# funcwj/setk

Measured on AMD Instinct MI355X. Metric: real-time-factor (audio-sec/wall-sec), 8-ch 16 kHz MVDR, higher is better.
Workload: dtype f32; 1 GPU; 8-ch 16 kHz oracle-mask MVDR, 30 s utterances, 125 per GPU (BASELINE configs[2] shard: 1000 at 8 GPUs), STFT 512/256/hann/center, inputs resident in HBM; utts_per_gpu=125, channels=8, frames=1876, beamformer=mvdr, parallelism=utterance-sharded x1

## Files before the change

setk_amd/csrc/capi_fused.hip:

```cpp
#include "capi.h"

using namespace setk;

extern "C" {

int setk_apply_weights_batch(setk_handle_t h, int n_utts, int num_channels,
                             const float* const* audio, const int* num_samples,
                             const float* weights, int n_sets, const int* weight_index,
                             void* const* wave, int flags, void* stream) {
    if (!h || n_utts <= 0 || !audio || !num_samples || !weights || n_sets <= 0 || !wave)
        return fail(h, SETK_ERR_INVALID, "bad args");
    SETK_TRY(require_plan512(h));
    const int C = num_channels;
    if (C < 1 || C > kMaxChannels) return fail(h, SETK_ERR_UNSUPPORTED, "1 <= num_channels <= 8");
    if (weight_index)
        for (int u = 0; u < n_utts; ++u)
            if (weight_index[u] < 0 || weight_index[u] >= n_sets)
                return fail(h, SETK_ERR_INVALID, "weight index out of range");
    hipStream_t s;
    SETK_TRY(begin_call(h, stream, &s));
    const bool pcm16 = (flags & SETK_FLAG_OUT_PCM16) != 0;

    std::vector<UttDesc> uds = zeroed_utts(n_utts);
    std::vector<WorkItem> items;
// ... 122 lines not shown
    memcpy(blob.data() + b_ud + b_i1, items2.data(), b_i2);
    if (blob != h->desc_cache) {
        if (blob.size() > h->d_desc_cap) {
            HIP_TRY(h, hipStreamSynchronize(s));
            if (h->d_desc) (void)hipFree(h->d_desc);
            h->d_desc = nullptr;
            h->d_desc_cap = 0;
            HIP_TRY(h, hipMalloc(reinterpret_cast<void**>(&h->d_desc), blob.size() * 2));
            h->d_desc_cap = blob.size() * 2;
        }
        HIP_TRY(h, h2d_small(h, h->d_desc, blob.data(), blob.size(), s));
        h->desc_cache.swap(blob);
    }
    const UttDesc* d_uds = reinterpret_cast<const UttDesc*>(h->d_desc);
    const WorkItem* d_items1 = reinterpret_cast<const WorkItem*>(h->d_desc + b_ud);
    const WorkItem* d_items2 = reinterpret_cast<const WorkItem*>(h->d_desc + b_ud + b_i1);

    const int planes_out = mpdr ? 6 * NP : 4 * NP;
    float *d_part, *d_covar, *d_w;
    unsigned* d_small;
    SETK_TRY(arena_get(h, (size_t)nparts_total * nplanes_partial(C) * kBinsPad * 4, &d_part));
    SETK_TRY(arena_get(h, (size_t)n_utts * planes_out * kBinsPad * 4, &d_covar));
    SETK_TRY(arena_get(h, (size_t)n_utts * C * kBinsPad * 8, &d_w));
    SETK_TRY(arena_get(h, (size_t)n_utts * 3 * 4, &d_small));
    unsigned* d_norm = d_small;
    unsigned* d_omax = d_small + n_utts;
    int* d_status = reinterpret_cast<int*>(d_small + 2 * n_utts);
    HIP_TRY(h, hipMemsetAsync(d_small, 0, (size_t)n_utts * 3 * 4, s));

    SETK_TRY(profile_begin(h, s));

    Pass1Args p1 = pass1_args(h, d_uds, d_items1);
    p1.partials = d_part;
    p1.norm_bits = d_norm;
    p1.flags = opts->flags;
    p1.mc_tab = h->d_mc_tab;
    p1.mc_win = h->d_mc_win;
    const bool mc1 = !in_pcm && h->mc_enabled && pass1_mc_supported(C, g.hop) && getenv("SETK_MC_PASS1") &&
                     atoi(getenv("SETK_MC_PASS1")) != 0;
    if (in_pcm) p1.window = h->d_window_pcm;
    if (mc1)
        HIP_TRY(h, launch_pass1_mc(C, p1, (int)items1.size(), s));
    else
        HIP_TRY(h, launch_pass1(C, false, p1, (int)items1.size(), s, in_pcm));
    SETK_TRY(profile_mark(h, 1, s));
    FinalizeArgs fa;
    memset(&fa, 0, sizeof(fa));
    fa.utts = d_uds;
    fa.partials = d_part;
    fa.covar = d_covar;
    fa.num_channels = C;
    fa.with_ry = mpdr ? 1 : 0;
    fa.num_scale = mc1 ? (float)((h->mc_peak / 1024.0) * (h->mc_peak / 1024.0)) : 1.f;
    const bool fuse_reduce = !(taps && (taps->Rs || taps->Rn)) && max_parts <= 4 &&
                             !(kind == SETK_BF_PMWF && opts->pmwf_ref < 0) &&
                             !(getenv("SETK_FUSED_REDUCE") && atoi(getenv("SETK_FUSED_REDUCE")) == 0);
    if (!fuse_reduce) HIP_TRY(h, launch_finalize(fa, n_utts, s));
    OutBuf tap_rs, tap_rn, tap_w;
    if (taps && taps->Rs) {
        SETK_TRY(stage_out(h, taps->Rs, (size_t)n_utts * kBins * C * C * sizeof(float2), &tap_rs));
        HIP_TRY(h, launch_unpack_covar(d_covar, n_utts, planes_out, 0, kBins, C,
                                       static_cast<float*>(tap_rs.dev), s));
        SETK_TRY(copy_back(h, tap_rs, s));
    }
    if (taps && taps->Rn) {
        SETK_TRY(stage_out(h, taps->Rn, (size_t)n_utts * kBins * C * C * sizeof(float2), &tap_rn));
        HIP_TRY(h, launch_unpack_covar(d_covar, n_utts, planes_out, 2 * NP, kBins, C,
                                       static_cast<float*>(tap_rn.dev), s));
        SETK_TRY(copy_back(h, tap_rn, s));
    }

    SolveArgs sa;
    memset(&sa, 0, sizeof(sa));
    sa.covar = d_covar;
    sa.weight = d_w;
    sa.status = d_status;
    sa.n_utts = n_utts;
    sa.num_bins = kBins;
    sa.num_channels = C;
    sa.planes = planes_out;
    sa.kind = kind;
    sa.flags = opts->flags;
    sa.rank1 = opts->rank1;
    sa.pmwf_ref = opts->pmwf_ref;
    sa.pmwf_beta = opts->pmwf_beta;
    sa.partials = fuse_reduce ? d_part : nullptr;
    sa.utts = d_uds;
    sa.num_scale = fa.num_scale;
    if (kind == SETK_BF_PMWF && opts->pmwf_ref < 0) {
        SETK_TRY(arena_get(h, (size_t)n_utts * kBins * C * 2 * sizeof(double), &sa.snr_acc));
        SETK_TRY(arena_get(h, (size_t)n_utts * kBins * C * C * 8, &sa.wmat));
    }
    HIP_TRY(h, launch_solve(sa, s));
    if (kind == SETK_BF_PMWF && opts->pmwf_ref < 0) HIP_TRY(h, launch_pmwf_select(sa, nullptr, s));
    SETK_TRY(profile_mark(h, 2, s));
    if (taps && taps->weight) {
        SETK_TRY(stage_out(h, taps->weight, (size_t)n_utts * kBins * C * sizeof(float2), &tap_w));
        HIP_TRY(h, launch_unpack_weight_batch(d_w, n_utts, kBins, C,
                                              static_cast<float*>(tap_w.dev), s));
        SETK_TRY(copy_back(h, tap_w, s));
    }

    Pass2Args p2 = pass2_args(h, d_uds, d_items2, d_omax);
    p2.weight = d_w;
    p2.norm_bits = d_norm;
    p2.flags = opts->flags;
    p2.mc_tab = h->d_mc_tab;
// ... 20 lines not shown
```

setk_amd/csrc/common.h:

```cpp
#pragma once
#include <hip/hip_runtime.h>
#include <stdint.h>

namespace setk {

constexpr int kNfft = 512;
constexpr int kBins = 257;
constexpr int kBinsPad = 264;
constexpr int kMaxChannels = 8;
constexpr int kMaxChannels16 = 16;
constexpr int kSuperTile = 16;
constexpr int kPass2Threads = 16 * kSuperTile;
constexpr int kPass2WavesPerSimd = 2;
constexpr int kMaxKeep = 7;

__host__ __device__ constexpr int npairs(int c) { return c * (c + 1) / 2; }
__host__ __device__ constexpr int pass1_tile_frames(int c) { return (32 / c) < 8 ? (32 / c) : 8; }
__host__ __device__ constexpr int nplanes_partial(int c) { return 4 * npairs(c) + 2; }
__host__ __device__ constexpr int pair_index(int i, int j, int c) {
    return i * c - i * (i - 1) / 2 + (j - i);
}

constexpr int kAudioF32 = 0;
constexpr int kAudioPcm16 = 1;

struct UttDesc {
    const float* audio;
    const float* mask_s;
    const float* mask_n;
    float* wave_f32;
    void* wave_out;
    int num_samples;
    int num_frames;
    int out_len;
    int part0;
    int nparts;
    int audio_fmt;
    int ch_stride;
    int pad_;
};

struct WorkItem {
    int utt;
    int t0, t1;
    int part;
    int last;
};

struct StftGeom {
    int hop;
    int pad;
    int center;
    int keep;
};

struct Pass1Args {
    const UttDesc* utts;
    const WorkItem* items;
    float* partials;
    const float* window;
    const float2* tw256;
    const float2* tw512;
    unsigned* norm_bits;
    float* spec_dump;
    int dump_pitch;
    StftGeom g;
    int flags;
    const unsigned* mc_tab;
    const float* mc_win;
};

struct FinalizeArgs {
    const UttDesc* utts;
    const float* partials;
    float* covar;
    int num_channels;
    int with_ry;
    float num_scale;
};

struct SolveArgs {
    const float* covar;
    float* weight;
    int* status;
    int* bin_status;
    double* snr_acc;
    float* wmat;
    int n_utts;
    int num_bins;
    int num_channels;
    int planes;
    int kind, flags, rank1, pmwf_ref;
    float pmwf_beta;
// ... 184 lines not shown
```

setk_amd/csrc/dpp.h:

```cpp
#pragma once
#include <hip/hip_runtime.h>

namespace setk {

#ifndef SD
#define SD __device__ __forceinline__
#endif

template <int M>
SD int dpp_xor(int v) {
    constexpr int qp[4] = {0, 0xB1, 0x4E, 0x1B};
    if constexpr (M < 4) {
        return __builtin_amdgcn_update_dpp(0, v, qp[M], 0xf, 0xf, true);
    } else if constexpr (M == 7) {
        return __builtin_amdgcn_update_dpp(0, v, 0x141, 0xf, 0xf, true);
    } else if constexpr (M < 8) {
        const int h = __builtin_amdgcn_update_dpp(0, v, 0x141, 0xf, 0xf, true);
        return __builtin_amdgcn_update_dpp(0, h, qp[M ^ 7], 0xf, 0xf, true);
    } else if constexpr (M == 8) {
        return __builtin_amdgcn_update_dpp(0, v, 0x128, 0xf, 0xf, true);
    } else if constexpr (M < 12) {
        const int h = __builtin_amdgcn_update_dpp(0, v, 0x128, 0xf, 0xf, true);
        return __builtin_amdgcn_update_dpp(0, h, qp[M ^ 8], 0xf, 0xf, true);
    } else if constexpr (M == 15) {
        return __builtin_amdgcn_update_dpp(0, v, 0x140, 0xf, 0xf, true);
    } else {
        const int h = __builtin_amdgcn_update_dpp(0, v, 0x140, 0xf, 0xf, true);
        return __builtin_amdgcn_update_dpp(0, h, qp[M ^ 15], 0xf, 0xf, true);
    }
}
template <int M>
SD double dshfl_xor(double x) {
    const long long b = __builtin_bit_cast(long long, x);
    const int lo = dpp_xor<M>((int)(b & 0xffffffffll));
    const int hi = dpp_xor<M>((int)(b >> 32));
    return __builtin_bit_cast(double, ((long long)hi << 32) | (unsigned int)lo);
}

}
```

setk_amd/csrc/solve.hip:

```cpp
#include "common.h"
#include "dpp.h"
#include <hip/hip_runtime.h>
#include "../../include/setk_hip.h"

namespace setk {

typedef double2 cd;

#define SD __device__ __forceinline__

SD cd zadd(cd a, cd b) { return make_double2(a.x + b.x, a.y + b.y); }
SD cd zsub(cd a, cd b) { return make_double2(a.x - b.x, a.y - b.y); }
SD cd zmul(cd a, cd b) { return make_double2(a.x * b.x - a.y * b.y, a.x * b.y + a.y * b.x); }
SD cd zmulc(cd a, cd b) { return make_double2(a.x * b.x + a.y * b.y, a.y * b.x - a.x * b.y); }
SD cd zcmul(cd a, cd b) { return make_double2(a.x * b.x + a.y * b.y, a.x * b.y - a.y * b.x); }
SD cd zscale(cd a, double s) { return make_double2(a.x * s, a.y * s); }
SD cd zdiv(cd a, cd b) {
    const double d = b.x * b.x + b.y * b.y;
    return make_double2((a.x * b.x + a.y * b.y) / d, (a.y * b.x - a.x * b.y) / d);
}
SD double zabs2(cd a) { return a.x * a.x + a.y * a.y; }
template <int C> struct Grp { static constexpr int W = (C > 8) ? 16 : (C > 4) ? 8 : 4; };
template <int W>
SD cd zshfl(cd v, int src) { return make_double2(__shfl(v.x, src, W), __shfl(v.y, src, W)); }

constexpr int kKindPevd = 100;
constexpr double kEpsF32 = 1.1920928955078125e-07;

template <int C, int M>
SD bool jacobi_round(cd (&g)[C], int j, double floor2) {
    const double tol2 = 1e-16;
    const int p = j ^ M;
    cd gp[C];
    double m = 0.0, o = 0.0, dyb = 0.0;
    cd d = make_double2(0.0, 0.0);
#pragma unroll
    for (int i = 0; i < C; ++i) {
        gp[i] = make_double2(dshfl_xor<M>(g[i].x), dshfl_xor<M>(g[i].y));
        m = fma(g[i].x, g[i].x, fma(g[i].y, g[i].y, m));
        o = fma(gp[i].x, gp[i].x, fma(gp[i].y, gp[i].y, o));
        d.x = fma(g[i].x, gp[i].x, fma(g[i].y, gp[i].y, d.x));
        d.y = fma(g[i].x, gp[i].y, d.y);
        dyb = fma(g[i].y, gp[i].x, dyb);
    }
    d.y -= dyb;
    const double dd = fma(d.x, d.x, d.y * d.y);
    if (dd > tol2 * (m * o) && dd > floor2) {
        const double absd = sqrt(dd);
        const double sigma = (j < p) ? 1.0 : -1.0;
        const double zeta = sigma * (o - m) / (2.0 * absd);
        const double t = copysign(1.0, zeta) / (fabs(zeta) + sqrt(1.0 + zeta * zeta));
        const double cs = 1.0 / sqrt(1.0 + t * t);
        const double sn = cs * t;
        const double f = sigma * sn / absd;
        const cd ph = make_double2(d.x * f, -d.y * f);
#pragma unroll
        for (int i = 0; i < C; ++i) g[i] = zsub(zscale(g[i], cs), zmul(ph, gp[i]));
        return true;
    }
    return false;
}

template <int C>
SD void jacobi_pevd(cd (&g)[C], int j, cd (&out)[C], double& lam, int& noconv) {
    constexpr int W = Grp<C>::W;
    bool done = false;
    for (int sweep = 0; sweep < 40 && !done; ++sweep) {
        double mm = 0.0;
#pragma unroll
        for (int i = 0; i < C; ++i) mm += zabs2(g[i]);
#pragma unroll
        for (int sft = 1; sft < W; sft <<= 1) mm = fmax(mm, __shfl_xor(mm, sft, W));
        const double floor2 = 1e-28 * mm * mm;
        bool rot = false;
        rot |= jacobi_round<C, 1>(g, j, floor2);
        rot |= jacobi_round<C, 2>(g, j, floor2);
        rot |= jacobi_round<C, 3>(g, j, floor2);
        if constexpr (W >= 8) {
            rot |= jacobi_round<C, 4>(g, j, floor2);
            rot |= jacobi_round<C, 5>(g, j, floor2);
            rot |= jacobi_round<C, 6>(g, j, floor2);
            rot |= jacobi_round<C, 7>(g, j, floor2);
        }
        if constexpr (W == 16) {
            rot |= jacobi_round<C, 8>(g, j, floor2);
            rot |= jacobi_round<C, 9>(g, j, floor2);
            rot |= jacobi_round<C, 10>(g, j, floor2);
            rot |= jacobi_round<C, 11>(g, j, floor2);
            rot |= jacobi_round<C, 12>(g, j, floor2);
            rot |= jacobi_round<C, 13>(g, j, floor2);
            rot |= jacobi_round<C, 14>(g, j, floor2);
            rot |= jacobi_round<C, 15>(g, j, floor2);
        }
        done = !__any(rot);
    }
    if (!done) noconv = 1;
    double m = 0.0;
#pragma unroll
    for (int i = 0; i < C; ++i) m += zabs2(g[i]);
    double best = m;
    int bj = j;
#pragma unroll
    for (int s = 1; s < W; s <<= 1) {
        const double ob = __shfl_xor(best, s, W);
        const int oj = __shfl_xor(bj, s, W);
        if (ob > best || (ob == best && oj < bj)) {
            best = ob;
            bj = oj;
        }
    }
    lam = sqrt(best);
    const double inv = (lam > 0.0) ? 1.0 / lam : 0.0;
#pragma unroll
    for (int i = 0; i < C; ++i) {
        out[i] = zscale(zshfl<W>(g[i], bj), inv);
        if (!(lam > 0.0)) out[i] = make_double2((i == 0) ? 1.0 : 0.0, 0.0);
    }
}

template <int C>
SD void herm_matvec(const cd (&col)[C], const cd (&x)[C], cd (&y)[C]) {
    cd mine = make_double2(0.0, 0.0);
#pragma unroll
    for (int m = 0; m < C; ++m) mine = zadd(mine, zcmul(col[m], x[m]));
#pragma unroll
    for (int i = 0; i < C; ++i) y[i] = zshfl<Grp<C>::W>(mine, i);
}

template <int M>
SD float fxor(float x) {
    return __builtin_bit_cast(float, dpp_xor<M>(__builtin_bit_cast(int, x)));
}
template <int C, int M>
SD bool jacobi_round_f32(float2 (&g)[C], int j, float floor2) {
    const float tol2 = 1e-11f;
    const int p = j ^ M;
    float2 gp[C];
    float m = 0.f;
    float2 d = make_float2(0.f, 0.f);
    float dyb = 0.f;
#pragma unroll
    for (int i = 0; i < C; ++i) {
        gp[i] = make_float2(fxor<M>(g[i].x), fxor<M>(g[i].y));
        m = fmaf(g[i].x, g[i].x, fmaf(g[i].y, g[i].y, m));
        d.x = fmaf(g[i].x, gp[i].x, fmaf(g[i].y, gp[i].y, d.x));
        d.y = fmaf(g[i].x, gp[i].y, d.y);
        dyb = fmaf(g[i].y, gp[i].x, dyb);
    }
    d.y -= dyb;
    const float o = fxor<M>(m);
    const float dd = fmaf(d.x, d.x, d.y * d.y);
    if (dd > tol2 * (m * o) && dd > floor2) {
        const float rabs = __builtin_amdgcn_rsqf(dd);
        const float sigma = (j < p) ? 1.f : -1.f;
        const float zeta = sigma * (o - m) * 0.5f * rabs;
        const float t = copysignf(1.f, zeta) / (fabsf(zeta) + sqrtf(fmaf(zeta, zeta, 1.f)));
        const float cs = __builtin_amdgcn_rsqf(fmaf(t, t, 1.f));
        const float f = sigma * cs * t * rabs;
        const float2 ph = make_float2(d.x * f, -d.y * f);
#pragma unroll
        for (int i = 0; i < C; ++i) {
            const float2 t0 = g[i];
            g[i].x = fmaf(t0.x, cs, fmaf(-ph.x, gp[i].x, ph.y * gp[i].y));
            g[i].y = fmaf(t0.y, cs, fmaf(-ph.x, gp[i].y, -ph.y * gp[i].x));
        }
        return true;
    }
    return false;
}

template <int C>
SD void pevd_mixed(const cd (&a)[C], int j, cd (&out)[C], double& lam, int& noconv) {
    constexpr int W = Grp<C>::W;
    if constexpr (W > 8) {
        cd g[C];
#pragma unroll
        for (int i = 0; i < C; ++i) g[i] = a[i];
        jacobi_pevd<C>(g, j, out, lam, noconv);
        return;
    } else {
        double dg = 0.0;
#pragma unroll
        for (int i = 0; i < C; ++i)
            if (i == j) dg = a[i].x;
#pragma unroll
        for (int s = 1; s < W; s <<= 1) dg = fmax(dg, __shfl_xor(dg, s, W));
        const double rs = (dg > 0.0) ? 1.0 / dg : 0.0;
        float2 g[C];
#pragma unroll
        for (int i = 0; i < C; ++i) g[i] = make_float2((float)(a[i].x * rs), (float)(a[i].y * rs));
        bool done = false;
        for (int sweep = 0; sweep < 40 && !done; ++sweep) {
            float mm = 0.f;
#pragma unroll
            for (int i = 0; i < C; ++i) mm = fmaf(g[i].x, g[i].x, fmaf(g[i].y, g[i].y, mm));
            mm = fmaxf(mm, fxor<1>(mm));
            mm = fmaxf(mm, fxor<2>(mm));
            if constexpr (W == 8) mm = fmaxf(mm, fxor<4>(mm));
            const float floor2 = 1e-12f * mm * mm;
            bool rot = false;
            rot |= jacobi_round_f32<C, 1>(g, j, floor2);
            rot |= jacobi_round_f32<C, 2>(g, j, floor2);
            rot |= jacobi_round_f32<C, 3>(g, j, floor2);
            if constexpr (W == 8) {
                rot |= jacobi_round_f32<C, 4>(g, j, floor2);
                rot |= jacobi_round_f32<C, 5>(g, j, floor2);
                rot |= jacobi_round_f32<C, 6>(g, j, floor2);
                rot |= jacobi_round_f32<C, 7>(g, j, floor2);
            }
            done = !__any(rot);
        }
        if (!done) noconv = 1;
        float m = 0.f;
#pragma unroll
        for (int i = 0; i < C; ++i) m = fmaf(g[i].x, g[i].x, fmaf(g[i].y, g[i].y, m));
        float best = m;
        int bj = j;
#pragma unroll
        for (int s = 1; s < W; s <<= 1) {
            const float ob = __shfl_xor(best, s, W);
            const int oj = __shfl_xor(bj, s, W);
            if (ob > best || (ob == best && oj < bj)) {
                best = ob;
                bj = oj;
            }
        }
        cd v[C];
        double nn = 0.0;
#pragma unroll
        for (int i = 0; i < C; ++i) {
            v[i] = make_double2((double)__shfl(g[i].x, bj, W), (double)__shfl(g[i].y, bj, W));
            nn += zabs2(v[i]);
        }
        double inv = (nn > 0.0) ? 1.0 / sqrt(nn) : 0.0;
#pragma unroll
        for (int i = 0; i < C; ++i) v[i] = zscale(v[i], inv);
        const double nj = sqrt((double)m);
        const double ij = (nj > 0.0) ? 1.0 / nj : 0.0;
        const double theta_j = nj * dg;
        cd y[C];
#pragma unroll 1
        for (int it = 0; it < 2; ++it) {
            herm_matvec<C>(a, v, y);
            double theta = 0.0;
#pragma unroll
            for (int i = 0; i < C; ++i) theta += zcmul(v[i], y[i]).x;
            cd c = make_double2(0.0, 0.0);
#pragma unroll
            for (int i = 0; i < C; ++i) {
                const cd u = make_double2((double)g[i].x * ij, (double)g[i].y * ij);
                c = zadd(c, zcmul(u, zsub(y[i], zscale(v[i], theta))));
            }
            const double den = theta - theta_j;
            const bool use = j != bj && nj > 0.0 && fabs(den) > 16.0 * kEpsF32 * fabs(theta);
            const cd coef = use ? zscale(c, 1.0 / den) : make_double2(0.0, 0.0);
            nn = 0.0;
#pragma unroll
            for (int i = 0; i < C; ++i) {
                cd t = zmul(make_double2((double)g[i].x * ij, (double)g[i].y * ij), coef);
#pragma unroll
                for (int sft = 1; sft < W; sft <<= 1) {
                    t.x += __shfl_xor(t.x, sft, W);
                    t.y += __shfl_xor(t.y, sft, W);
                }
                v[i] = zadd(v[i], t);
                nn += zabs2(v[i]);
            }
            inv = (nn > 0.0) ? 1.0 / sqrt(nn) : 0.0;
#pragma unroll
            for (int i = 0; i < C; ++i) v[i] = zscale(v[i], inv);
        }
        herm_matvec<C>(a, v, y);
        nn = 0.0;
#pragma unroll
        for (int i = 0; i < C; ++i) nn += zabs2(y[i]);
        lam = sqrt(nn);
        inv = (lam > 0.0) ? 1.0 / lam : 0.0;
#pragma unroll
        for (int i = 0; i < C; ++i) v[i] = zscale(y[i], inv);
#pragma unroll
        for (int i = 0; i < C; ++i) {
            out[i] = v[i];
            if (!(lam > 0.0)) out[i] = make_double2((i == 0) ? 1.0 : 0.0, 0.0);
        }
    }
}

template <int C>
SD void fix_gauge(cd (&v)[C]) {
    const double a = sqrt(zabs2(v[0]));
    if (a > 0.0) {
        const cd ph = make_double2(v[0].x / a, -v[0].y / a);
#pragma unroll
        for (int i = 0; i < C; ++i) v[i] = zmul(v[i], ph);
        v[0].y = 0.0;
    }
}

template <int C>
SD int chol_lds(const cd (&col)[C], cd* L, double* piv, int j, bool zero_is_identity = false) {
    double diag = 0.0;
#pragma unroll
    for (int i = 0; i < C; ++i)
        if (i == j) diag = col[i].x;
    double scale = diag;
#pragma unroll
    for (int s = 1; s < Grp<C>::W; s <<= 1) scale = fmax(scale, __shfl_xor(scale, s, Grp<C>::W));
    if (zero_is_identity && scale == 0.0) {
#pragma unroll
        for (int k = 0; k < C; ++k)
            if (j >= k && j < C) L[k * C + j] = make_double2(j == k ? 1.0 : 0.0, 0.0);
        __syncthreads();
        return 0;
    }
    const int bad0 = !(scale > 0.0);
    int bad = bad0;
    const double floor_piv = kEpsF32 * scale;
    double load = 0.0;
    for (int attempt = 0; attempt < 2; ++attempt) {
        bool hit = false;
        bad = bad0;
#pragma unroll
        for (int k = 0; k < C; ++k) {
            cd s = make_double2(0.0, 0.0);
            if (j >= k && j < C) {
                s = make_double2(col[k].x, -col[k].y);
                if (j == k) s.x += load;
                for (int m = 0; m < k; ++m) s = zsub(s, zmulc(L[m * C + j], L[m * C + k]));
            }
            if (j == k) *piv = s.x;
            __syncthreads();
            double d = *piv;
            if (!(d == d)) bad = 1;
            if (!(d >= floor_piv)) hit = true;
            d = fmax(d, floor_piv);
            const double rd = (d > 0.0) ? 1.0 / sqrt(d) : 0.0;
            if (j >= k && j < C) L[k * C + j] = (j == k) ? make_double2(d * rd, 0.0) : zscale(s, rd);
            __syncthreads();
        }
        if (attempt == 1 || !__any(hit && !bad0)) break;
        load = (hit && !bad0) ? 8.0 * floor_piv : 0.0;
    }
    return bad;
}

template <int C>
SD void fwd_solve(const cd* L, cd (&b)[C]) {
#pragma unroll
    for (int k = 0; k < C; ++k) {
        const double r = 1.0 / L[k * C + k].x;
        b[k] = zscale(b[k], r);
#pragma unroll
        for (int i = k + 1; i < C; ++i) b[i] = zsub(b[i], zmul(L[k * C + i], b[k]));
        __builtin_amdgcn_sched_barrier(0);
    }
}
template <int C>
SD void bwd_solve(const cd* L, cd (&y)[C]) {
#pragma unroll
    for (int k = C - 1; k >= 0; --k) {
        cd s = y[k];
#pragma unroll
        for (int i = k + 1; i < C; ++i) s = zsub(s, zcmul(L[k * C + i], y[i]));
        y[k] = zscale(s, 1.0 / L[k * C + k].x);
        __builtin_amdgcn_sched_barrier(0);
    }
}

template <int W>
SD double group_sum(double v) {
#pragma unroll
    for (int s = 1; s < W; s <<= 1) v += __shfl_xor(v, s, W);
    return v;
}

template <int C>
SD void gev_vector(const cd (&rs)[C], const cd* L, cd* Wk, int j, bool gauge, cd (&vout)[C],
                   int& noconv) {
    cd x[C];
#pragma unroll
    for (int i = 0; i < C; ++i) x[i] = rs[i];
    fwd_solve<C>(L, x);
    __syncthreads();
    if (j < C) {
#pragma unroll
        for (int i = 0; i < C; ++i) Wk[j * C + i] = x[i];
    }
    __syncthreads();
    cd c[C];
#pragma unroll
    for (int m = 0; m < C; ++m) {
        const cd t = (j < C) ? Wk[m * C + j] : make_double2(0.0, 0.0);
        c[m] = make_double2(t.x, -t.y);
    }
    fwd_solve<C>(L, c);
    if (j >= C) {
#pragma unroll
        for (int i = 0; i < C; ++i) c[i] = make_double2(0.0, 0.0);
    }
    cd y[C];
    double lam;
    pevd_mixed<C>(c, j, y, lam, noconv);
    if (gauge) fix_gauge<C>(y);
    bwd_solve<C>(L, y);
#pragma unroll
    for (int i = 0; i < C; ++i) vout[i] = y[i];
}

template <int C, int KIND>
__global__ __launch_bounds__(64, (C > 8) ? 1 : 2) void solve_kernel(SolveArgs a, int pitch, int lds_mats) {
    constexpr int NP = npairs(C);
    constexpr int W = Grp<C>::W;
    constexpr int PW = 64 / W;
    extern __shared__ __attribute__((aligned(16))) char solve_smem[];
    cd* mats = reinterpret_cast<cd*>(solve_smem);
    double* sPiv = reinterpret_cast<double*>(mats + (size_t)lds_mats * PW * C * C);

    const int tid = threadIdx.x;
    const int j = tid & (W - 1), q = tid / W;
    const int F = a.num_bins;
    const long n_prob = (long)a.n_utts * F;
    long prob = (long)blockIdx.x * PW + q;
    const bool live = prob < n_prob;
    if (!live) prob = n_prob - 1;
    const int u = (int)(prob / F), f = (int)(prob % F);

    cd* L = mats + ((size_t)0 * PW + q) * C * C;
    cd* Wk = mats + ((size_t)(lds_mats > 1 ? 1 : 0) * PW + q) * C * C;
    cd* Rsf = mats + ((size_t)(lds_mats > 2 ? 2 : 0) * PW + q) * C * C;
    cd* Rnf = mats + ((size_t)(lds_mats > 3 ? 3 : 0) * PW + q) * C * C;
    double* piv = &sPiv[q];

    constexpr int kind = KIND;
    const bool gauge = (a.flags & SETK_FLAG_NO_GAUGE) == 0;
    const bool have_rn = a.planes >= 4 * NP && kind != SETK_BF_MPDR;

    const float* base = a.covar + (size_t)u * a.planes * pitch + f;
    const bool fused = a.partials != nullptr;
    const int planes_in = 4 * NP + 2;
    const size_t slab = (size_t)planes_in * pitch;
    const float* P = nullptr;
    int nparts = 0;
    float scale_of[3] = {0.f, 0.f, 0.f};
    if (fused) {
        const UttDesc ud = a.utts[u];
        P = a.partials + (size_t)ud.part0 * slab + f;
        nparts = ud.nparts;
        float den0 = 0.f, den1 = 0.f;
        for (int p = 0; p < nparts; ++p) {
            den0 += P[p * slab + (size_t)(4 * NP + 0) * pitch];
            den1 += P[p * slab + (size_t)(4 * NP + 1) * pitch];
        }
        scale_of[0] = a.num_scale / fmaxf(den0, 1e-6f);
        scale_of[1] = a.num_scale / fmaxf(den1, 1e-6f);
        scale_of[2] = a.num_scale / fmaxf((float)ud.num_frames, 1e-6f);
    }
    bool finite = true;
    auto load_col = [&](int which, cd (&m)[C]) {
#pragma unroll
        for (int i = 0; i < C; ++i) {
            m[i] = make_double2(0.0, 0.0);
            if (j < C) {
                const int lo = i < j ? i : j, hi = i < j ? j : i;
                const int e = pair_index(lo, hi, C);
                const double sgn = (i <= j) ? 1.0 : -1.0;
                float re, im;
                if (!fused) {
                    re = base[(size_t)((2 * which + 0) * NP + e) * pitch];
                    im = base[(size_t)((2 * which + 1) * NP + e) * pitch];
                } else if (which < 2) {
                    float ar = 0.f, ai = 0.f;
                    for (int p = 0; p < nparts; ++p) {
                        ar += P[p * slab + (size_t)((2 * which + 0) * NP + e) * pitch];
                        ai += P[p * slab + (size_t)((2 * which + 1) * NP + e) * pitch];
                    }
                    re = ar * scale_of[which];
                    im = ai * scale_of[which];
                } else {
                    float ar = 0.f, ai = 0.f;
                    for (int p = 0; p < nparts; ++p) {
                        ar += P[p * slab + (size_t)(0 * NP + e) * pitch] + P[p * slab + (size_t)(2 * NP + e) * pitch];
                        ai += P[p * slab + (size_t)(1 * NP + e) * pitch] + P[p * slab + (size_t)(3 * NP + e) * pitch];
                    }
                    re = ar * scale_of[2];
                    im = ai * scale_of[2];
                }
                m[i] = make_double2(re, (i == j) ? 0.0 : sgn * im);
                finite = finite && isfinite(re) && isfinite(im);
            }
        }
    };

    int st_sing = 0, st_noconv = 0;
    cd w[C];
#pragma unroll
    for (int i = 0; i < C; ++i) w[i] = make_double2(0.0, 0.0);

    if (kind == kKindPevd && !have_rn) {
        cd g[C];
        load_col(0, g);
        double lam;
        pevd_mixed<C>(g, j, w, lam, st_noconv);
        if (gauge) fix_gauge<C>(w);
    } else if (kind == kKindPevd || kind == SETK_BF_GEVD) {
        {
            cd rn[C];
            load_col(1, rn);
            st_sing |= chol_lds<C>(rn, L, piv, j,
                                   kind == SETK_BF_GEVD && (a.flags & SETK_FLAG_STRICT_REFERENCE) != 0);
        }
        cd rs[C];
        load_col(0, rs);
        gev_vector<C>(rs, L, Wk, j, gauge, w, st_noconv);
    } else if (kind == SETK_BF_MVDR) {
        cd d[C];
        {
            cd g[C];
            load_col(0, g);
            double lam;
            pevd_mixed<C>(g, j, d, lam, st_noconv);
        }
        if (gauge) fix_gauge<C>(d);
        {
            cd rn[C];
            load_col(1, rn);
            st_sing |= chol_lds<C>(rn, L, piv, j);
        }
        cd num[C];
#pragma unroll
        for (int i = 0; i < C; ++i) num[i] = d[i];
        fwd_solve<C>(L, num);
        bwd_solve<C>(L, num);
        cd den = make_double2(0.0, 0.0);
#pragma unroll
        for (int i = 0; i < C; ++i) den = zadd(den, zcmul(d[i], num[i]));
#pragma unroll
        for (int i = 0; i < C; ++i) w[i] = zdiv(num[i], den);
    } else if (kind == SETK_BF_MPDR || kind == SETK_BF_MPDR_WHITEN) {
        cd sv[C];
        if (kind == SETK_BF_MPDR) {
            cd g[C];
            load_col(0, g);
            double lam;
            pevd_mixed<C>(g, j, sv, lam, st_noconv);
            if (gauge) fix_gauge<C>(sv);
        } else {
            cd rn[C];
            load_col(1, rn);
            st_sing |= chol_lds<C>(rn, L, piv, j);
            cd v[C];
            {
                cd rs[C];
                load_col(0, rs);
                gev_vector<C>(rs, L, Wk, j, gauge, v, st_noconv);
            }
            herm_matvec<C>(rn, v, sv);
            __syncthreads();
        }
        {
            cd ry[C];
            load_col(2, ry);
            st_sing |= chol_lds<C>(ry, L, piv, j);
        }
        cd num[C];
#pragma unroll
        for (int i = 0; i < C; ++i) num[i] = sv[i];
        fwd_solve<C>(L, num);
        bwd_solve<C>(L, num);
        cd den = make_double2(0.0, 0.0);
#pragma unroll
        for (int i = 0; i < C; ++i) den = zadd(den, zcmul(sv[i], num[i]));
#pragma unroll
        for (int i = 0; i < C; ++i) w[i] = zdiv(num[i], den);
    } else if (kind == SETK_BF_PMWF) {
        cd rs[C], rn[C];
        load_col(0, rs);
        load_col(1, rn);
        st_sing |= chol_lds<C>(rn, L, piv, j);
        if (a.rank1 != SETK_RANK1_NONE) {
            cd pv[C];
            if (a.rank1 == SETK_RANK1_EIG) {
                cd g[C];
#pragma unroll
                for (int i = 0; i < C; ++i) g[i] = rs[i];
                double lam;
                pevd_mixed<C>(g, j, pv, lam, st_noconv);
            } else {
                cd v[C];
                gev_vector<C>(rs, L, Wk, j, false, v, st_noconv);
                herm_matvec<C>(rn, v, pv);
            }
            double dj = 0.0, pn = 0.0;
#pragma unroll
            for (int i = 0; i < C; ++i) {
                if (i == j) dj = rs[i].x;
                pn += zabs2(pv[i]);
            }
            const double tr = group_sum<Grp<C>::W>(dj);
            const double sc = tr / fmax(pn, kEpsF32);
            cd pj = make_double2(0.0, 0.0);
#pragma unroll
            for (int i = 0; i < C; ++i)
                if (i == j) pj = pv[i];
#pragma unroll
            for (int i = 0; i < C; ++i)
                rs[i] = (j < C) ? zscale(zmulc(pv[i], pj), sc) : make_double2(0.0, 0.0);
        }
        cd x[C];
#pragma unroll
        for (int i = 0; i < C; ++i) x[i] = rs[i];
        fwd_solve<C>(L, x);
        bwd_solve<C>(L, x);
        cd diag = make_double2(0.0, 0.0);
#pragma unroll
        for (int i = 0; i < C; ++i)
            if (i == j) diag = x[i];
        cd den = make_double2(group_sum<Grp<C>::W>(diag.x) + (double)a.pmwf_beta, group_sum<Grp<C>::W>(diag.y));
#pragma unroll
        for (int i = 0; i < C; ++i) x[i] = zdiv(x[i], den);
        if (a.pmwf_ref >= 0) {
#pragma unroll
            for (int i = 0; i < C; ++i) w[i] = zshfl<Grp<C>::W>(x[i], a.pmwf_ref);
        } else {
            __syncthreads();
            if (j < C) {
#pragma unroll
                for (int i = 0; i < C; ++i) {
                    Rsf[j * C + i] = rs[i];
                    Rnf[j * C + i] = rn[i];
                }
            }
            __syncthreads();
            double ps = 0.0, pn = 0.0, nb = 0.0;
#pragma unroll
            for (int i = 0; i < C; ++i) {
                cd s1 = make_double2(0.0, 0.0), s2 = s1;
#pragma unroll
                for (int m = 0; m < C; ++m) {
                    s1 = zadd(s1, zmul(Rsf[m * C + i], x[m]));
                    s2 = zadd(s2, zmul(Rnf[m * C + i], x[m]));
                }
                ps += zcmul(x[i], s1).x;
                pn += zcmul(x[i], s2).x;
                nb += zabs2(s2);
            }
            const double filt = (a.flags & SETK_FLAG_BAN) ? sqrt(nb) / fmax(pn, kEpsF32) : 1.0;
            if (live && j < C) {
                a.snr_acc[((size_t)prob * C + j) * 2 + 0] = ps;
                a.snr_acc[((size_t)prob * C + j) * 2 + 1] = pn;
                float2* wm = reinterpret_cast<float2*>(a.wmat) + ((size_t)prob * C + j) * C;
#pragma unroll
                for (int i = 0; i < C; ++i) wm[i] = make_float2((float)(x[i].x * filt), (float)(x[i].y * filt));
            }
        }
    }

    if ((a.flags & SETK_FLAG_BAN) && !(kind == SETK_BF_PMWF && a.pmwf_ref < 0)) {
        cd rn[C];
#pragma unroll
        for (int i = 0; i < C; ++i) rn[i] = make_double2(0.0, 0.0);
        if (have_rn) load_col(1, rn);
        cd uj = make_double2(0.0, 0.0);
        cd wj = make_double2(0.0, 0.0);
#pragma unroll
        for (int m = 0; m < C; ++m) uj = zadd(uj, zcmul(rn[m], w[m]));
#pragma unroll
        for (int i = 0; i < C; ++i)
            if (i == j) wj = w[i];
        const double nom = group_sum<Grp<C>::W>(zabs2(uj));
        const double den = group_sum<Grp<C>::W>(zcmul(wj, uj).x);
        const double filt = sqrt(nom) / fmax(den, kEpsF32);
#pragma unroll
        for (int i = 0; i < C; ++i) w[i] = zscale(w[i], filt);
    }

    int st = SETK_NUM_OK;
    if (st_noconv) st = SETK_NUM_NOCONV;
    if (st_sing) st = SETK_NUM_SINGULAR;
    bool wfin = true;
#pragma unroll
    for (int i = 0; i < C; ++i) wfin = wfin && isfinite(w[i].x) && isfinite(w[i].y);
    int fin = finite ? 1 : 0;
#pragma unroll
    for (int sft = 1; sft < W; sft <<= 1) fin &= __shfl_xor(fin, sft, W);
    if (!fin || (!wfin && st == SETK_NUM_OK)) st = SETK_NUM_NONFINITE;
    if (live) {
        if (j < C && !(kind == SETK_BF_PMWF && a.pmwf_ref < 0)) {
            cd wj = make_double2(0.0, 0.0);
#pragma unroll
            for (int i = 0; i < C; ++i)
                if (i == j) wj = w[i];
            float2* dst = reinterpret_cast<float2*>(a.weight) + ((size_t)u * C + j) * pitch + f;
            *dst = make_float2((float)wj.x, (float)wj.y);
        }
        if (j == 0) {
            if (a.bin_status) a.bin_status[prob] = st;
            if (a.status && st) atomicMax(a.status + u, st);
        }
    }
}


#pragma clang fp contract(off)
template <int CM>
__global__ __launch_bounds__(64) void lu_refusal_kernel(SolveArgs a, int pitch, int which) {
    const int C = a.num_channels, F = a.num_bins;
    const int NP = npairs(C);
    const long n_prob = (long)a.n_utts * F;
    const long prob = (long)blockIdx.x * 64 + threadIdx.x;
    if (prob >= n_prob) return;
    const int u = (int)(prob / F), f = (int)(prob % F);
    float ar[CM][CM], ai[CM][CM];
    const bool fused = a.partials != nullptr;
    const size_t slab = (size_t)(4 * NP + 2) * pitch;
    const float* base = a.covar + (size_t)u * a.planes * pitch + f;
    const float* P = nullptr;
    int nparts = 0;
    float scale = 0.f;
    if (fused) {
        const UttDesc ud = a.utts[u];
        P = a.partials + (size_t)ud.part0 * slab + f;
        nparts = ud.nparts;
        float den = 0.f;
        if (which < 2) {
            for (int p = 0; p < nparts; ++p) den += P[p * slab + (size_t)(4 * NP + which) * pitch];
        } else {
            den = (float)ud.num_frames;
        }
        scale = a.num_scale / fmaxf(den, 1e-6f);
    }
    for (int i = 0; i < C; ++i)
        for (int k = i; k < C; ++k) {
            const int e = pair_index(i, k, C);
            float re, im;
            if (!fused) {
                re = base[(size_t)((2 * which + 0) * NP + e) * pitch];
                im = base[(size_t)((2 * which + 1) * NP + e) * pitch];
// ... 18 lines not shown
            ai[k][i] = -im;
        }
    bool singular = false;
    for (int k = 0; k < C && !singular; ++k) {
        int p = k;
        float best = fabsf(ar[k][k]) + fabsf(ai[k][k]);
        for (int i = k + 1; i < C; ++i) {
            const float v = fabsf(ar[i][k]) + fabsf(ai[i][k]);
            if (v > best) {
                best = v;
                p = i;
            }
        }
        if (best == 0.f) {
            singular = true;
            break;
        }
        if (p != k)
            for (int m = 0; m < C; ++m) {
                const float tr = ar[k][m], ti = ai[k][m];
                ar[k][m] = ar[p][m];
                ai[k][m] = ai[p][m];
                ar[p][m] = tr;
                ai[p][m] = ti;
            }
        const float pr = ar[k][k], pi = ai[k][k];
        const float d = pr * pr + pi * pi;
        for (int i = k + 1; i < C; ++i) {
            const float lr = (ar[i][k] * pr + ai[i][k] * pi) / d;
            const float li = (ai[i][k] * pr - ar[i][k] * pi) / d;
            for (int m = k + 1; m < C; ++m) {
                ar[i][m] = ar[i][m] - (lr * ar[k][m] - li * ai[k][m]);
                ai[i][m] = ai[i][m] - (lr * ai[k][m] + li * ar[k][m]);
            }
        }
    }
    if (singular) {
        if (a.bin_status) atomicMax(a.bin_status + prob, SETK_NUM_SINGULAR);
        if (a.status) atomicMax(a.status + u, SETK_NUM_SINGULAR);
    }
}
#pragma clang fp contract(fast)

hipError_t launch_solve(const SolveArgs& a, hipStream_t s) {
    const long n_prob = (long)a.n_utts * a.num_bins;
    const int pw = a.num_channels > 8 ? 4 : (a.num_channels > 4 ? 8 : 16);
    const int blocks = (int)((n_prob + pw - 1) / pw);
    const int pitch = (a.num_bins == kBins) ? kBinsPad : ((a.num_bins + 7) / 8) * 8;
    int lds_mats = 2;
    if (a.kind == SETK_BF_MVDR || a.kind == SETK_BF_MPDR) lds_mats = 1;
    if (a.kind == SETK_BF_PMWF) lds_mats = 4;
#define SETK_LAUNCH(c, k)                                                              \
    do {                                                                               \
        const size_t lds = (size_t)lds_mats * pw * c * c * sizeof(cd) + pw * sizeof(double); \
        if (lds > (64u << 10)) {                                                       \
            hipError_t e = hipFuncSetAttribute(                                        \
                reinterpret_cast<const void*>(solve_kernel<c, k>),                     \
                hipFuncAttributeMaxDynamicSharedMemorySize, (int)lds);                 \
            if (e != hipSuccess) return e;                                             \
        }                                                                              \
        hipLaunchKernelGGL((solve_kernel<c, k>), dim3(blocks), dim3(64), lds, s, a,    \
                           pitch, lds_mats);                                           \
    } while (0)
#define SETK_CASE(c)                                                                   \
    case c:                                                                            \
        switch (a.kind) {                                                              \
            case SETK_BF_MVDR: SETK_LAUNCH(c, SETK_BF_MVDR); break;                    \
            case SETK_BF_GEVD: SETK_LAUNCH(c, SETK_BF_GEVD); break;                    \
            case SETK_BF_PMWF: SETK_LAUNCH(c, SETK_BF_PMWF); break;                    \
            case SETK_BF_MPDR: SETK_LAUNCH(c, SETK_BF_MPDR); break;                    \
            case SETK_BF_MPDR_WHITEN: SETK_LAUNCH(c, SETK_BF_MPDR_WHITEN); break;      \
            case kKindPevd: SETK_LAUNCH(c, kKindPevd); break;                          \
            default: return hipErrorInvalidValue;                                      \
        }                                                                              \
        break;
    switch (a.num_channels) {
        SETK_CASE(1)
        SETK_CASE(2)
        SETK_CASE(3)
        SETK_CASE(4)
        SETK_CASE(5)
        SETK_CASE(6)
        SETK_CASE(7)
        SETK_CASE(8)
        SETK_CASE(16)
        default:
            return hipErrorInvalidValue;
    }
#undef SETK_CASE
#undef SETK_LAUNCH
    hipError_t e = hipGetLastError();
    if (e != hipSuccess) return e;
    if ((a.flags & SETK_FLAG_STRICT_REFERENCE) &&
        (a.kind == SETK_BF_MVDR || a.kind == SETK_BF_PMWF || a.kind == SETK_BF_MPDR ||
         a.kind == SETK_BF_MPDR_WHITEN)) {
        const int which = (a.kind == SETK_BF_MVDR || a.kind == SETK_BF_PMWF) ? 1 : 2;
        const dim3 grid((unsigned)((n_prob + 63) / 64));
        if (a.num_channels <= 4) hipLaunchKernelGGL(lu_refusal_kernel<4>, grid, dim3(64), 0, s, a, pitch, which);
        else if (a.num_channels <= 8) hipLaunchKernelGGL(lu_refusal_kernel<8>, grid, dim3(64), 0, s, a, pitch, which);
        else hipLaunchKernelGGL(lu_refusal_kernel<kMaxChannels16>, grid, dim3(64), 0, s, a, pitch, which);
        e = hipGetLastError();
    }
    return e;
}

__global__ __launch_bounds__(256) void pmwf_select_kernel(SolveArgs a, int pitch, int* ref_out) {
    const int u = blockIdx.y;
// ... 219 lines not shown
```

Before: 2.170 million x real time (audio seconds per wall second, all GPUs).

## Use DPP group reductions and broadcasts in solve; prefetch noise covariance

Replaces __shfl_xor-based group reductions and broadcasts in the per-bin solve kernel with DPP lane ops. The Cholesky pivot is now broadcast through DPP instead of an LDS slot plus a barrier, which removes one __syncthreads per column and the pivot LDS slot. The partial-sum loads for the fused reduce are unrolled to a fixed maximum part count, and in MVDR the noise covariance loads are issued before the eigenvector iteration so their latency overlaps that compute. The cost is higher register pressure from holding the raw columns across the eigen solve, and the code now assumes max_parts is at most kFuseMaxParts.

```diff
diff --git a/setk_amd/csrc/capi_fused.hip b/setk_amd/csrc/capi_fused.hip
--- a/setk_amd/csrc/capi_fused.hip
+++ b/setk_amd/csrc/capi_fused.hip
@@ -198,7 +198,7 @@
     fa.num_channels = C;
     fa.with_ry = mpdr ? 1 : 0;
     fa.num_scale = mc1 ? (float)((h->mc_peak / 1024.0) * (h->mc_peak / 1024.0)) : 1.f;
-    const bool fuse_reduce = !(taps && (taps->Rs || taps->Rn)) && max_parts <= 4 &&
+    const bool fuse_reduce = !(taps && (taps->Rs || taps->Rn)) && max_parts <= kFuseMaxParts &&
                              !(kind == SETK_BF_PMWF && opts->pmwf_ref < 0) &&
                              !(getenv("SETK_FUSED_REDUCE") && atoi(getenv("SETK_FUSED_REDUCE")) == 0);
     if (!fuse_reduce) HIP_TRY(h, launch_finalize(fa, n_utts, s));
diff --git a/setk_amd/csrc/common.h b/setk_amd/csrc/common.h
--- a/setk_amd/csrc/common.h
+++ b/setk_amd/csrc/common.h
@@ -39,6 +39,8 @@
     int ch_stride;
     int pad_;
 };
+
+constexpr int kFuseMaxParts = 4;
 
 struct WorkItem {
     int utt;
diff --git a/setk_amd/csrc/dpp.h b/setk_amd/csrc/dpp.h
--- a/setk_amd/csrc/dpp.h
+++ b/setk_amd/csrc/dpp.h
@@ -37,4 +37,58 @@
     return __builtin_bit_cast(double, ((long long)hi << 32) | (unsigned int)lo);
 }
 
+template <int M>
+SD float fshfl_xor(float x) {
+    return __builtin_bit_cast(float, dpp_xor<M>(__builtin_bit_cast(int, x)));
 }
+template <int M> SD int lane_xor(int x) { return dpp_xor<M>(x); }
+template <int M> SD float lane_xor(float x) { return fshfl_xor<M>(x); }
+template <int M> SD double lane_xor(double x) { return dshfl_xor<M>(x); }
+
+template <int W, class T, class Op>
+SD T group_fold(T v, Op op) {
+    v = op(v, lane_xor<1>(v));
+    v = op(v, lane_xor<2>(v));
+    if constexpr (W >= 8) v = op(v, lane_xor<4>(v));
+    if constexpr (W >= 16) v = op(v, lane_xor<8>(v));
+    return v;
+}
+template <int W> SD double group_sum(double v) { return group_fold<W>(v, [](double a, double b) { return a + b; }); }
+template <int W> SD double group_max(double v) { return group_fold<W>(v, [](double a, double b) { return fmax(a, b); }); }
+template <int W> SD float group_max(float v) { return group_fold<W>(v, [](float a, float b) { return fmaxf(a, b); }); }
+template <int W> SD int group_and(int v) { return group_fold<W>(v, [](int a, int b) { return a & b; }); }
+template <int W, class T>
+SD void group_argmax(T& best, int& bj) {
+    auto step = [&](T ob, int oj) {
+        if (ob > best || (ob == best && oj < bj)) {
+            best = ob;
+            bj = oj;
+        }
+    };
+    step(lane_xor<1>(best), lane_xor<1>(bj));
+    step(lane_xor<2>(best), lane_xor<2>(bj));
+    if constexpr (W >= 8) step(lane_xor<4>(best), lane_xor<4>(bj));
+    if constexpr (W >= 16) step(lane_xor<8>(best), lane_xor<8>(bj));
+}
+
+template <int W, int I>
+SD int dpp_bcast(int v) {
+    static_assert(I >= 0 && I < W && (W == 4 || W == 8 || W == 16), "lane of a 4-, 8- or 16-lane group");
+    if constexpr (W == 4) {
+        return __builtin_amdgcn_update_dpp(0, v, I * 0x55, 0xf, 0xf, true);
+    } else if constexpr (W == 16) {
+        return __builtin_amdgcn_update_dpp(0, v, 0x150 + I, 0xf, 0xf, true);
+    } else {
+        const int lo = __builtin_amdgcn_update_dpp(0, v, 0x150 + I, 0xf, 0x3, false);
+        return __builtin_amdgcn_update_dpp(lo, v, 0x158 + I, 0xf, 0xc, false);
+    }
+}
+template <int W, int I>
+SD double dbcast(double x) {
+    const long long b = __builtin_bit_cast(long long, x);
+    const int lo = dpp_bcast<W, I>((int)(b & 0xffffffffll));
+    const int hi = dpp_bcast<W, I>((int)(b >> 32));
+    return __builtin_bit_cast(double, ((long long)hi << 32) | (unsigned int)lo);
+}
+
+}
diff --git a/setk_amd/csrc/solve.hip b/setk_amd/csrc/solve.hip
--- a/setk_amd/csrc/solve.hip
+++ b/setk_amd/csrc/solve.hip
@@ -1,6 +1,7 @@
 #include "common.h"
 #include "dpp.h"
 #include <hip/hip_runtime.h>
+#include <type_traits>
 #include "../../include/setk_hip.h"
 
 namespace setk {
@@ -69,8 +70,7 @@
         double mm = 0.0;
 #pragma unroll
         for (int i = 0; i < C; ++i) mm += zabs2(g[i]);
-#pragma unroll
-        for (int sft = 1; sft < W; sft <<= 1) mm = fmax(mm, __shfl_xor(mm, sft, W));
+        mm = group_max<W>(mm);
         const double floor2 = 1e-28 * mm * mm;
         bool rot = false;
         rot |= jacobi_round<C, 1>(g, j, floor2);
@@ -100,15 +100,7 @@
     for (int i = 0; i < C; ++i) m += zabs2(g[i]);
     double best = m;
     int bj = j;
-#pragma unroll
-    for (int s = 1; s < W; s <<= 1) {
-        const double ob = __shfl_xor(best, s, W);
-        const int oj = __shfl_xor(bj, s, W);
-        if (ob > best || (ob == best && oj < bj)) {
-            best = ob;
-            bj = oj;
-        }
-    }
+    group_argmax<W>(best, bj);
     lam = sqrt(best);
     const double inv = (lam > 0.0) ? 1.0 / lam : 0.0;
 #pragma unroll
@@ -118,19 +110,27 @@
     }
 }
 
+template <int N, int I = 0, class F>
+SD void static_for(F&& f) {
+    if constexpr (I < N) {
+        f(std::integral_constant<int, I>{});
+        static_for<N, I + 1>(f);
+    }
+}
+
 template <int C>
 SD void herm_matvec(const cd (&col)[C], const cd (&x)[C], cd (&y)[C]) {
     cd mine = make_double2(0.0, 0.0);
 #pragma unroll
     for (int m = 0; m < C; ++m) mine = zadd(mine, zcmul(col[m], x[m]));
-#pragma unroll
-    for (int i = 0; i < C; ++i) y[i] = zshfl<Grp<C>::W>(mine, i);
+    static_for<C>([&](auto ic) {
+        constexpr int i = decltype(ic)::value;
+        y[i] = make_double2(dbcast<Grp<C>::W, i>(mine.x), dbcast<Grp<C>::W, i>(mine.y));
+    });
 }
 
 template <int M>
-SD float fxor(float x) {
-    return __builtin_bit_cast(float, dpp_xor<M>(__builtin_bit_cast(int, x)));
-}
+SD float fxor(float x) { return fshfl_xor<M>(x); }
 template <int C, int M>
 SD bool jacobi_round_f32(float2 (&g)[C], int j, float floor2) {
     const float tol2 = 1e-11f;
@@ -183,8 +183,7 @@
 #pragma unroll
         for (int i = 0; i < C; ++i)
             if (i == j) dg = a[i].x;
-#pragma unroll
-        for (int s = 1; s < W; s <<= 1) dg = fmax(dg, __shfl_xor(dg, s, W));
+        dg = group_max<W>(dg);
         const double rs = (dg > 0.0) ? 1.0 / dg : 0.0;
         float2 g[C];
 #pragma unroll
@@ -194,9 +193,7 @@
             float mm = 0.f;
 #pragma unroll
             for (int i = 0; i < C; ++i) mm = fmaf(g[i].x, g[i].x, fmaf(g[i].y, g[i].y, mm));
-            mm = fmaxf(mm, fxor<1>(mm));
-            mm = fmaxf(mm, fxor<2>(mm));
-            if constexpr (W == 8) mm = fmaxf(mm, fxor<4>(mm));
+            mm = group_max<W>(mm);
             const float floor2 = 1e-12f * mm * mm;
             bool rot = false;
             rot |= jacobi_round_f32<C, 1>(g, j, floor2);
@@ -216,15 +213,7 @@
         for (int i = 0; i < C; ++i) m = fmaf(g[i].x, g[i].x, fmaf(g[i].y, g[i].y, m));
         float best = m;
         int bj = j;
-#pragma unroll
-        for (int s = 1; s < W; s <<= 1) {
-            const float ob = __shfl_xor(best, s, W);
-            const int oj = __shfl_xor(bj, s, W);
-            if (ob > best || (ob == best && oj < bj)) {
-                best = ob;
-                bj = oj;
-            }
-        }
+        group_argmax<W>(best, bj);
         cd v[C];
         double nn = 0.0;
 #pragma unroll
@@ -258,11 +247,7 @@
 #pragma unroll
             for (int i = 0; i < C; ++i) {
                 cd t = zmul(make_double2((double)g[i].x * ij, (double)g[i].y * ij), coef);
-#pragma unroll
-                for (int sft = 1; sft < W; sft <<= 1) {
-                    t.x += __shfl_xor(t.x, sft, W);
-                    t.y += __shfl_xor(t.y, sft, W);
-                }
+                t = make_double2(group_sum<W>(t.x), group_sum<W>(t.y));
                 v[i] = zadd(v[i], t);
                 nn += zabs2(v[i]);
             }
@@ -298,14 +283,12 @@
 }
 
 template <int C>
-SD int chol_lds(const cd (&col)[C], cd* L, double* piv, int j, bool zero_is_identity = false) {
+SD int chol_lds(const cd (&col)[C], cd* L, int j, bool zero_is_identity = false) {
     double diag = 0.0;
 #pragma unroll
     for (int i = 0; i < C; ++i)
         if (i == j) diag = col[i].x;
-    double scale = diag;
-#pragma unroll
-    for (int s = 1; s < Grp<C>::W; s <<= 1) scale = fmax(scale, __shfl_xor(scale, s, Grp<C>::W));
+    const double scale = group_max<Grp<C>::W>(diag);
     if (zero_is_identity && scale == 0.0) {
 #pragma unroll
         for (int k = 0; k < C; ++k)
@@ -320,24 +303,22 @@
     for (int attempt = 0; attempt < 2; ++attempt) {
         bool hit = false;
         bad = bad0;
-#pragma unroll
-        for (int k = 0; k < C; ++k) {
+        static_for<C>([&](auto kc) {
+            constexpr int k = decltype(kc)::value;
             cd s = make_double2(0.0, 0.0);
             if (j >= k && j < C) {
                 s = make_double2(col[k].x, -col[k].y);
                 if (j == k) s.x += load;
                 for (int m = 0; m < k; ++m) s = zsub(s, zmulc(L[m * C + j], L[m * C + k]));
             }
-            if (j == k) *piv = s.x;
-            __syncthreads();
-            double d = *piv;
+            double d = dbcast<Grp<C>::W, k>(s.x);
             if (!(d == d)) bad = 1;
             if (!(d >= floor_piv)) hit = true;
             d = fmax(d, floor_piv);
             const double rd = (d > 0.0) ? 1.0 / sqrt(d) : 0.0;
             if (j >= k && j < C) L[k * C + j] = (j == k) ? make_double2(d * rd, 0.0) : zscale(s, rd);
             __syncthreads();
-        }
+        });
         if (attempt == 1 || !__any(hit && !bad0)) break;
         load = (hit && !bad0) ? 8.0 * floor_piv : 0.0;
     }
@@ -365,13 +346,6 @@
         y[k] = zscale(s, 1.0 / L[k * C + k].x);
         __builtin_amdgcn_sched_barrier(0);
     }
-}
-
-template <int W>
-SD double group_sum(double v) {
-#pragma unroll
-    for (int s = 1; s < W; s <<= 1) v += __shfl_xor(v, s, W);
-    return v;
 }
 
 template <int C>
@@ -414,7 +388,6 @@
     constexpr int PW = 64 / W;
     extern __shared__ __attribute__((aligned(16))) char solve_smem[];
     cd* mats = reinterpret_cast<cd*>(solve_smem);
-    double* sPiv = reinterpret_cast<double*>(mats + (size_t)lds_mats * PW * C * C);
 
     const int tid = threadIdx.x;
     const int j = tid & (W - 1), q = tid / W;
@@ -429,7 +402,6 @@
     cd* Wk = mats + ((size_t)(lds_mats > 1 ? 1 : 0) * PW + q) * C * C;
     cd* Rsf = mats + ((size_t)(lds_mats > 2 ? 2 : 0) * PW + q) * C * C;
     cd* Rnf = mats + ((size_t)(lds_mats > 3 ? 3 : 0) * PW + q) * C * C;
-    double* piv = &sPiv[q];
 
     constexpr int kind = KIND;
     const bool gauge = (a.flags & SETK_FLAG_NO_GAUGE) == 0;
@@ -447,16 +419,82 @@
         P = a.partials + (size_t)ud.part0 * slab + f;
         nparts = ud.nparts;
         float den0 = 0.f, den1 = 0.f;
-        for (int p = 0; p < nparts; ++p) {
-            den0 += P[p * slab + (size_t)(4 * NP + 0) * pitch];
-            den1 += P[p * slab + (size_t)(4 * NP + 1) * pitch];
-        }
+        float d0[kFuseMaxParts], d1[kFuseMaxParts];
+#pragma unroll
+        for (int p = 0; p < kFuseMaxParts; ++p) {
+            const int pp = p < nparts ? p : 0;
+            d0[p] = P[pp * slab + (size_t)(4 * NP + 0) * pitch];
+            d1[p] = P[pp * slab + (size_t)(4 * NP + 1) * pitch];
+        }
+#pragma unroll
+        for (int p = 0; p < kFuseMaxParts; ++p)
+            if (p < nparts) {
+                den0 += d0[p];
+                den1 += d1[p];
+            }
         scale_of[0] = a.num_scale / fmaxf(den0, 1e-6f);
         scale_of[1] = a.num_scale / fmaxf(den1, 1e-6f);
         scale_of[2] = a.num_scale / fmaxf((float)ud.num_frames, 1e-6f);
     }
     bool finite = true;
+    struct RawCol {
+        float re[kFuseMaxParts][C], im[kFuseMaxParts][C];
+    };
+    auto request_col = [&](int which, RawCol& r) {
+        auto fetch = [&](const float* src, float (&re)[C], float (&im)[C]) {
+#pragma unroll
+            for (int i = 0; i < C; ++i) {
+                re[i] = im[i] = 0.f;
+                if (j < C) {
+                    const int lo = i < j ? i : j, hi = i < j ? j : i;
+                    const int e = pair_index(lo, hi, C);
+                    re[i] = src[(size_t)((2 * which + 0) * NP + e) * pitch];
+                    im[i] = src[(size_t)((2 * which + 1) * NP + e) * pitch];
+                }
+            }
+        };
+        if (!fused) {
+            fetch(base, r.re[0], r.im[0]);
+        } else {
+#pragma unroll
+            for (int p = 0; p < kFuseMaxParts; ++p)
+                if (p < nparts) fetch(P + p * slab, r.re[p], r.im[p]);
+        }
+    };
+    auto finish_col = [&](int which, const RawCol& r, cd (&m)[C]) {
+#pragma unroll
+        for (int i = 0; i < C; ++i) {
+            m[i] = make_double2(0.0, 0.0);
+            if (j < C) {
+                const double sgn = (i <= j) ? 1.0 : -1.0;
+                float re, im;
+                if (!fused) {
+                    re = r.re[0][i];
+                    im = r.im[0][i];
+                } else {
+                    float ar = 0.f, ai = 0.f;
+#pragma unroll
+                    for (int p = 0; p < kFuseMaxParts; ++p)
+                        if (p < nparts) {
+                            ar += r.re[p][i];
+                            ai += r.im[p][i];
+                        }
+                    re = ar * scale_of[which];
+                    im = ai * scale_of[which];
+                }
+                m[i] = make_double2(re, (i == j) ? 0.0 : sgn * im);
+                finite = finite && isfinite(re) && isfinite(im);
+            }
+        }
+    };
+
     auto load_col = [&](int which, cd (&m)[C]) {
+        if (which < 2) {
+            RawCol r;
+            request_col(which, r);
+            finish_col(which, r, m);
+            return;
+        }
 #pragma unroll
         for (int i = 0; i < C; ++i) {
             m[i] = make_double2(0.0, 0.0);
@@ -466,16 +504,8 @@
                 const double sgn = (i <= j) ? 1.0 : -1.0;
                 float re, im;
                 if (!fused) {
-                    re = base[(size_t)((2 * which + 0) * NP + e) * pitch];
-                    im = base[(size_t)((2 * which + 1) * NP + e) * pitch];
-                } else if (which < 2) {
-                    float ar = 0.f, ai = 0.f;
-                    for (int p = 0; p < nparts; ++p) {
-                        ar += P[p * slab + (size_t)((2 * which + 0) * NP + e) * pitch];
-                        ai += P[p * slab + (size_t)((2 * which + 1) * NP + e) * pitch];
-                    }
-                    re = ar * scale_of[which];
-                    im = ai * scale_of[which];
+                    re = base[(size_t)(4 * NP + e) * pitch];
+                    im = base[(size_t)(5 * NP + e) * pitch];
                 } else {
                     float ar = 0.f, ai = 0.f;
                     for (int p = 0; p < nparts; ++p) {
@@ -506,7 +536,7 @@
         {
             cd rn[C];
             load_col(1, rn);
-            st_sing |= chol_lds<C>(rn, L, piv, j,
+            st_sing |= chol_lds<C>(rn, L, j,
                                    kind == SETK_BF_GEVD && (a.flags & SETK_FLAG_STRICT_REFERENCE) != 0);
         }
         cd rs[C];
@@ -514,17 +544,19 @@
         gev_vector<C>(rs, L, Wk, j, gauge, w, st_noconv);
     } else if (kind == SETK_BF_MVDR) {
         cd d[C];
+        RawCol rn_raw;
         {
             cd g[C];
             load_col(0, g);
+            request_col(1, rn_raw);
             double lam;
             pevd_mixed<C>(g, j, d, lam, st_noconv);
         }
         if (gauge) fix_gauge<C>(d);
         {
             cd rn[C];
-            load_col(1, rn);
-            st_sing |= chol_lds<C>(rn, L, piv, j);
+            finish_col(1, rn_raw, rn);
+            st_sing |= chol_lds<C>(rn, L, j);
         }
         cd num[C];
 #pragma unroll
@@ -547,7 +579,7 @@
         } else {
             cd rn[C];
             load_col(1, rn);
-            st_sing |= chol_lds<C>(rn, L, piv, j);
+            st_sing |= chol_lds<C>(rn, L, j);
             cd v[C];
             {
                 cd rs[C];
@@ -560,7 +592,7 @@
         {
             cd ry[C];
             load_col(2, ry);
-            st_sing |= chol_lds<C>(ry, L, piv, j);
+            st_sing |= chol_lds<C>(ry, L, j);
         }
         cd num[C];
 #pragma unroll
@@ -576,7 +608,7 @@
         cd rs[C], rn[C];
         load_col(0, rs);
         load_col(1, rn);
-        st_sing |= chol_lds<C>(rn, L, piv, j);
+        st_sing |= chol_lds<C>(rn, L, j);
         if (a.rank1 != SETK_RANK1_NONE) {
             cd pv[C];
             if (a.rank1 == SETK_RANK1_EIG) {
@@ -680,9 +712,7 @@
     bool wfin = true;
 #pragma unroll
     for (int i = 0; i < C; ++i) wfin = wfin && isfinite(w[i].x) && isfinite(w[i].y);
-    int fin = finite ? 1 : 0;
-#pragma unroll
-    for (int sft = 1; sft < W; sft <<= 1) fin &= __shfl_xor(fin, sft, W);
+    const int fin = group_and<W>(finite ? 1 : 0);
     if (!fin || (!wfin && st == SETK_NUM_OK)) st = SETK_NUM_NONFINITE;
     if (live) {
         if (j < C && !(kind == SETK_BF_PMWF && a.pmwf_ref < 0)) {
@@ -807,7 +837,7 @@
     if (a.kind == SETK_BF_PMWF) lds_mats = 4;
 #define SETK_LAUNCH(c, k)                                                              \
     do {                                                                               \
-        const size_t lds = (size_t)lds_mats * pw * c * c * sizeof(cd) + pw * sizeof(double); \
+        const size_t lds = (size_t)lds_mats * pw * c * c * sizeof(cd);                 \
         if (lds > (64u << 10)) {                                                       \
             hipError_t e = hipFuncSetAttribute(                                        \
                 reinterpret_cast<const void*>(solve_kernel<c, k>),                     \
```

New measurement: 2.185 million x real time (audio seconds per wall second, all GPUs) (median of 6 runs). Within noise of the previous version (+0.7%).
